# OpenBMB/VisRAG

Hardware: NVIDIA H100
Metric: page-images encoded/sec (higher is better)
Workload: dtype bf16

## Files before the change

visrag_b200/csrc/attention.cu:

```cuda
#include <string.h>
#include "common.h"
#include "attention.cuh"

namespace vr {

static int g_variant = 0;

template <int HS, bool CAUSAL, int NWG, bool F16>
static int launch_attention(const vr_attn_params& p, cudaStream_t stream) {
    using Cfg = AttCfg<HS, NWG>;
    AttMaps maps;
    memset(&maps, 0, sizeof(maps));
    const uint64_t qcols = p.ldq, kcols = p.ldk, vcols = p.ldv;
    if (int rc = make_tmap_2d(&maps.q64, p.q, p.q_rows, qcols, p.ldq, Cfg::BM, 64, 128, !F16)) return rc;
    if (int rc = make_tmap_2d(&maps.k64, p.k, p.kv_rows, kcols, p.ldk, ATT_BN, 64, 128, !F16)) return rc;
    if (int rc = make_tmap_2d(&maps.v64, p.v, p.kv_rows, vcols, p.ldv, ATT_BN, 64, 128, !F16)) return rc;
    if (Cfg::HAS16) {
        if (int rc = make_tmap_2d(&maps.q16, p.q, p.q_rows, qcols, p.ldq, Cfg::BM, 16, 32, !F16)) return rc;
        if (int rc = make_tmap_2d(&maps.k16, p.k, p.kv_rows, kcols, p.ldk, ATT_BN, 16, 32, !F16)) return rc;
        if (int rc = make_tmap_2d(&maps.v16, p.v, p.kv_rows, vcols, p.ldv, ATT_BN, 16, 32, !F16)) return rc;
    }
    AttArgs a;
    a.q_col0 = p.q_col0; a.k_col0 = p.k_col0; a.v_col0 = p.v_col0;
    a.head_dim = p.head_dim; a.heads = p.heads; a.batch = p.batch;
    a.cu_q = p.cu_q; a.cu_k = p.cu_k; a.max_q = p.max_q;
    a.scale_log2 = p.scale * 1.4426950408889634f;
    a.out = p.out;
    a.ldo = p.ldo;
    auto kern = attention_wgmma_kernel<HS, CAUSAL, NWG, F16>;
    static unsigned long long attr_set = 0;
    if (first_use_on_device(&attr_set))
        VR_CHECK_CUDA(cudaFuncSetAttribute(kern, cudaFuncAttributeMaxDynamicSharedMemorySize, Cfg::SMEM_BYTES));
    dim3 grid((p.max_q + Cfg::BM - 1) / Cfg::BM, p.heads, p.batch);
    kern<<<grid, Cfg::THREADS, Cfg::SMEM_BYTES, stream>>>(maps, a);
    VR_CHECK_CUDA(cudaGetLastError());
    return 0;
}

template <int HS, bool F16>
static int dispatch_attention(const vr_attn_params& p, cudaStream_t s) {
    const bool two = p.max_q > 64 && g_variant != 1;
    if (p.causal) return two ? launch_attention<HS, true, 2, F16>(p, s) : launch_attention<HS, true, 1, F16>(p, s);
    return two ? launch_attention<HS, false, 2, F16>(p, s) : launch_attention<HS, false, 1, F16>(p, s);
}

template <int HS>
static int dispatch_attention(const vr_attn_params& p, cudaStream_t s) {
    return (p.flags & VR_ATTN_F16) ? dispatch_attention<HS, true>(p, s) : dispatch_attention<HS, false>(p, s);
}

}

extern "C" void vr_attention_force_v1(int32_t variant) { vr::g_variant = variant; }

extern "C" int vr_attention(const vr_attn_params* p, void* stream) {
    using namespace vr;
    VR_REQUIRE(p && p->q && p->k && p->v && p->out && p->cu_k, "vr_attention: null pointer argument");
    VR_REQUIRE(p->heads > 0 && p->batch > 0 && p->max_q > 0 && p->max_k > 0, "vr_attention: empty problem");
    VR_REQUIRE(p->batch <= 65535 && p->heads <= 65535, "vr_attention: batch/heads exceed grid limits");
    VR_REQUIRE(p->head_dim <= p->head_stride && p->head_dim % 8 == 0, "vr_attention: head_dim %d vs stride %d",
               p->head_dim, p->head_stride);
    VR_REQUIRE(p->ldo % 8 == 0, "vr_attention: ldo must be a multiple of 8");
    VR_REQUIRE(!(p->flags & VR_ATTN_V_ONES_COLUMN) || p->head_dim == p->head_stride - 8,
               "vr_attention: VR_ATTN_V_ONES_COLUMN needs head_dim == head_stride - 8 (got %d / %d)", p->head_dim, p->head_stride);
    VR_REQUIRE_ALIGNED("vr_attention", "q", p->q, 16);
    VR_REQUIRE_ALIGNED("vr_attention", "k", p->k, 16);
    VR_REQUIRE_ALIGNED("vr_attention", "v", p->v, 16);
    VR_REQUIRE_ALIGNED("vr_attention", "cu_q", p->cu_q, 4);
    VR_REQUIRE_ALIGNED("vr_attention", "cu_k", p->cu_k, 4);
    VR_REQUIRE_ALIGNED("vr_attention", "out", p->out, 4);
    cudaStream_t s = reinterpret_cast<cudaStream_t>(stream);
    switch (p->head_stride) {
        case 64: return dispatch_attention<64>(*p, s);
        case 80: return dispatch_attention<80>(*p, s);
        case 128: return dispatch_attention<128>(*p, s);
        default: set_error("vr_attention: head_stride must be 64, 80 or 128 (got %d)", p->head_stride); return 2;
    }
}
```

visrag_b200/csrc/attention.cuh:

```cuda
#pragma once
#include "ptx.cuh"
#include "../../include/visrag_b200.h"

namespace vr {

constexpr int ATT_BN = 128;
constexpr int ATT_STAGES = 2;

template <int HS, int NWG>
struct AttCfg {
    static constexpr int BM = 64 * NWG;
    static constexpr int THREADS = 384;
    static constexpr int NCH = HS / 64;
    static constexpr bool HAS16 = (HS % 64) == 16;
    static_assert(HS == 64 || HS == 80 || HS == 128, "head stride must be 64, 80 or 128");
    static constexpr int Q_CHUNK = BM * 128;
    static constexpr int Q_BYTES = NCH * Q_CHUNK + (HAS16 ? BM * 32 : 0);
    static constexpr int TILE_BYTES = NCH * 16384 + (HAS16 ? 4096 : 0);
    static constexpr int OFF_Q = 0;
    static constexpr int OFF_K = (Q_BYTES + 1023) & ~1023;
    static constexpr int OFF_V = OFF_K + ATT_STAGES * TILE_BYTES;
    static constexpr int OFF_BAR = OFF_V + ATT_STAGES * TILE_BYTES;
    static constexpr int SMEM_BYTES = OFF_BAR + 128 + 1024;
};

struct AttArgs {
    int q_col0, k_col0, v_col0;
    int head_dim;
    int heads, batch;
    const int* cu_q;
    const int* cu_k;
    int max_q;
    float scale_log2;
    void* out;
    long long ldo;
};

struct AttMaps {
    CUtensorMap q64, q16, k64, k16, v64, v16;
};

template <bool F16, int NCH, bool HAS16>
__device__ __forceinline__ void att_store(const AttArgs& a, const float (&o)[NCH][32], const float (&o16)[8], float l_a, float l_b,
                                          int row_a, int len_q, int q_begin, int b, int head, int q4) {
    l_a += __shfl_xor_sync(0xffffffffu, l_a, 1);
    l_a += __shfl_xor_sync(0xffffffffu, l_a, 2);
    l_b += __shfl_xor_sync(0xffffffffu, l_b, 1);
    l_b += __shfl_xor_sync(0xffffffffu, l_b, 2);
#pragma unroll
    for (int half = 0; half < 2; ++half) {
        const int q_idx = row_a + 8 * half;
        if (q_idx >= len_q) continue;
        const float inv = 1.0f / (half ? l_b : l_a);
        const long long row = a.cu_q ? (long long)(q_begin + q_idx) : (long long)b * a.max_q + q_idx;
        half16_t<F16>* dst = reinterpret_cast<half16_t<F16>*>(a.out) + row * a.ldo + head * a.head_dim;
#pragma unroll
        for (int c = 0; c < NCH; ++c)
#pragma unroll
            for (int j = 0; j < 8; ++j) {
                const int col = c * 64 + j * 8 + q4 * 2;
                if (col < a.head_dim)
                    *reinterpret_cast<uint32_t*>(dst + col) = pack16x2<F16>(o[c][4 * j + 2 * half] * inv, o[c][4 * j + 2 * half + 1] * inv);
            }
        if (HAS16) {
#pragma unroll
            for (int j = 0; j < 2; ++j) {
                const int col = NCH * 64 + j * 8 + q4 * 2;
                if (col < a.head_dim)
                    *reinterpret_cast<uint32_t*>(dst + col) = pack16x2<F16>(o16[4 * j + 2 * half] * inv, o16[4 * j + 2 * half + 1] * inv);
            }
        }
    }
}

__device__ __forceinline__ void att_softmax_tile(float (&s)[64], float c, float& m_a, float& m_b, float& l_a, float& l_b,
                                                 float& alpha_a, float& alpha_b) {
    float mt_a = m_a, mt_b = m_b;
#pragma unroll
    for (int j = 0; j < 16; ++j) {
        mt_a = fmaxf(mt_a, fmaxf(s[4 * j], s[4 * j + 1]));
        mt_b = fmaxf(mt_b, fmaxf(s[4 * j + 2], s[4 * j + 3]));
    }
    mt_a = fmaxf(mt_a, __shfl_xor_sync(0xffffffffu, mt_a, 1));
    mt_a = fmaxf(mt_a, __shfl_xor_sync(0xffffffffu, mt_a, 2));
    mt_b = fmaxf(mt_b, __shfl_xor_sync(0xffffffffu, mt_b, 1));
    mt_b = fmaxf(mt_b, __shfl_xor_sync(0xffffffffu, mt_b, 2));
    const float mc_a = mt_a == -INFINITY ? 0.f : __fmul_rn(mt_a, c), mc_b = mt_b == -INFINITY ? 0.f : __fmul_rn(mt_b, c);
    alpha_a = ex2_ftz(__fmul_rn(m_a, c) - mc_a);
    alpha_b = ex2_ftz(__fmul_rn(m_b, c) - mc_b);
    m_a = mt_a;
    m_b = mt_b;
    float lt_a = 0.f, lt_b = 0.f;
#pragma unroll
    for (int j = 0; j < 16; ++j) {
#pragma unroll
        for (int e = 0; e < 2; ++e) {
            s[4 * j + e] = ex2_ftz(__fmaf_rn(s[4 * j + e], c, -mc_a));
            s[4 * j + 2 + e] = ex2_ftz(__fmaf_rn(s[4 * j + 2 + e], c, -mc_b));
            lt_a += s[4 * j + e];
            lt_b += s[4 * j + 2 + e];
        }
    }
    l_a = l_a * alpha_a + lt_a;
    l_b = l_b * alpha_b + lt_b;
}

template <int HS, bool CAUSAL, int NWG, bool F16>
__global__ void __launch_bounds__(384, 1)
attention_wgmma_kernel(const __grid_constant__ AttMaps maps, const AttArgs a) {
    using Cfg = AttCfg<HS, NWG>;
    constexpr int NCH = Cfg::NCH;
    extern __shared__ uint8_t smem_raw[];
    uint8_t* smem = reinterpret_cast<uint8_t*>((reinterpret_cast<uintptr_t>(smem_raw) + 1023) & ~uintptr_t(1023));
    uint8_t* sQ = smem + Cfg::OFF_Q;
    uint8_t* sK = smem + Cfg::OFF_K;
    uint8_t* sV = smem + Cfg::OFF_V;
    uint64_t* bars = reinterpret_cast<uint64_t*>(smem + Cfg::OFF_BAR);
    uint64_t* q_bar = bars + 0;
    uint64_t* k_full = bars + 1;
    uint64_t* k_empty = k_full + ATT_STAGES;
    uint64_t* v_full = k_empty + ATT_STAGES;
    uint64_t* v_empty = v_full + ATT_STAGES;
    uint64_t* v_tail = v_empty + ATT_STAGES;

    const int wg = threadIdx.x >> 7;
    const int warp = (threadIdx.x >> 5) & 3;
    const int lane = threadIdx.x & 31;
    const int qt = blockIdx.x, head = blockIdx.y, b = blockIdx.z;

    const int k_begin = a.cu_k[b];
    const int len_k = a.cu_k[b + 1] - k_begin;
    const int q_begin = a.cu_q ? a.cu_q[b] : 0;
    const int len_q = a.cu_q ? a.cu_q[b + 1] - q_begin : a.max_q;
    const int q0 = qt * Cfg::BM;
    if (q0 >= len_q || len_k <= 0) return;

    int nkt = (len_k + ATT_BN - 1) / ATT_BN;
    if (CAUSAL) {
        const int last_q = min(q0 + Cfg::BM, len_q) - 1;
        const int max_key = last_q + (len_k - len_q);
        nkt = min(nkt, max_key / ATT_BN + 1);
    }

    if (threadIdx.x == 0) {
        mbar_init(q_bar, 1);
        for (int i = 0; i < ATT_STAGES; ++i) {
            mbar_init(&k_full[i], 1);
            mbar_init(&v_full[i], 1);
            mbar_init(&k_empty[i], NWG * 4);
            mbar_init(&v_empty[i], NWG * 4);
        }
        mbar_init(v_tail, 1);
        fence_mbar_init();
    }
    __syncthreads();

    if (wg == 0 || wg > NWG) {
        setmaxnreg_dec<40>();
        if (wg == 0 && warp == 0) {
            const int tail = len_k - (nkt - 1) * ATT_BN;
            const int st_last = (nkt - 1) % ATT_STAGES;
            if (lane == 0) {
                const int qcol = a.q_col0 + head * HS, kcol = a.k_col0 + head * HS, vcol = a.v_col0 + head * HS;
                mbar_expect_tx(q_bar, Cfg::Q_BYTES);
#pragma unroll
                for (int c = 0; c < NCH; ++c) tma_load_2d(&maps.q64, q_bar, sQ + c * Cfg::Q_CHUNK, qcol + c * 64, q_begin + q0);
                if (Cfg::HAS16) tma_load_2d(&maps.q16, q_bar, sQ + NCH * Cfg::Q_CHUNK, qcol + NCH * 64, q_begin + q0);
                auto load_tile = [&](const CUtensorMap* m64, const CUtensorMap* m16, uint64_t* bar, uint8_t* dst, int col, int row) {
                    mbar_expect_tx(bar, Cfg::TILE_BYTES);
#pragma unroll
                    for (int c = 0; c < NCH; ++c) tma_load_2d(m64, bar, dst + c * 16384, col + c * 64, row);
                    if (Cfg::HAS16) tma_load_2d(m16, bar, dst + NCH * 16384, col + NCH * 64, row);
                };
                for (int kt = 0; kt < nkt; ++kt) {
                    const int st = kt % ATT_STAGES;
                    const uint32_t ph = (kt / ATT_STAGES) & 1;
                    mbar_wait(&k_empty[st], ph ^ 1);
                    load_tile(&maps.k64, &maps.k16, &k_full[st], sK + st * Cfg::TILE_BYTES, kcol, k_begin + kt * ATT_BN);
                    mbar_wait(&v_empty[st], ph ^ 1);
                    load_tile(&maps.v64, &maps.v16, kt == nkt - 1 && tail < ATT_BN ? v_tail : &v_full[st],
                              sV + st * Cfg::TILE_BYTES, vcol, k_begin + kt * ATT_BN);
                }
            }
            __syncwarp();
            if (tail < ATT_BN) {
                uint8_t* dst = sV + st_last * Cfg::TILE_BYTES;
                const uint4 zero = make_uint4(0u, 0u, 0u, 0u);
                mbar_wait(v_tail, 0);
#pragma unroll
                for (int c = 0; c < NCH; ++c)
                    for (int i = tail * 8 + lane; i < ATT_BN * 8; i += 32) reinterpret_cast<uint4*>(dst + c * 16384)[i] = zero;
                if (Cfg::HAS16)
                    for (int i = tail * 2 + lane; i < ATT_BN * 2; i += 32) reinterpret_cast<uint4*>(dst + NCH * 16384)[i] = zero;
                fence_proxy_async_smem();
                __syncwarp();
                if (lane == 0) mbar_arrive(&v_full[st_last]);
            }
        }
        return;
    }

    setmaxnreg_inc<232>();
    const int cw = wg - 1;
    const int g8 = lane >> 2, q4 = lane & 3;
    const int row_a = q0 + cw * 64 + warp * 16 + g8;
    const int row_b = row_a + 8;
    const int causal_shift = len_k - len_q;
    const uint32_t q_addr = smem_u32(sQ) + cw * (64 * 128);
    const uint32_t q16_addr = smem_u32(sQ) + NCH * Cfg::Q_CHUNK + cw * (64 * 32);

    if constexpr (NWG == 2 && HS != 128) {
        const float c = a.scale_log2;
        float o[NCH][32];
        float o16[8];
#pragma unroll
        for (int cc = 0; cc < NCH; ++cc)
#pragma unroll
            for (int j = 0; j < 32; ++j) o[cc][j] = 0.f;
#pragma unroll
        for (int j = 0; j < 8; ++j) o16[j] = 0.f;
        float m_a = -INFINITY, m_b = -INFINITY, l_a = 0.f, l_b = 0.f, alpha_a, alpha_b;
        float s[64];
        uint32_t pa[ATT_BN / 16][4];

        auto issue_s = [&](int kt) {
            const uint32_t k_addr = smem_u32(sK) + (kt % ATT_STAGES) * Cfg::TILE_BYTES;
#pragma unroll
            for (int cc = 0; cc < NCH; ++cc) {
#pragma unroll
                for (int kk = 0; kk < 4; ++kk)
                    wgmma_ss<F16, false>(s, make_smem_desc(q_addr + cc * Cfg::Q_CHUNK + kk * 32, 16, 1024, kLayoutSW128),
                                           make_smem_desc(k_addr + cc * 16384 + kk * 32, 16, 1024, kLayoutSW128), (cc | kk) != 0,
                                           std::integral_constant<int, 128>());
            }
            if (Cfg::HAS16)
                wgmma_ss<F16, false>(s, make_smem_desc(q16_addr, 16, 256, kLayoutSW32),
                                       make_smem_desc(k_addr + NCH * 16384, 16, 256, kLayoutSW32), 1, std::integral_constant<int, 128>());
            wgmma_commit();
        };
        auto issue_pv = [&](int kt) {
            const uint32_t v_addr = smem_u32(sV) + (kt % ATT_STAGES) * Cfg::TILE_BYTES;
#pragma unroll
            for (int kk = 0; kk < ATT_BN / 16; ++kk) {
#pragma unroll
                for (int cc = 0; cc < NCH; ++cc)
                    wgmma_rs_tb<F16>(o[cc], pa[kk], make_smem_desc(v_addr + cc * 16384 + kk * 2048, 16, 1024, kLayoutSW128), 1,
                                std::integral_constant<int, 64>());
                if (Cfg::HAS16)
                    wgmma_rs_tb<F16>(o16, pa[kk], make_smem_desc(v_addr + NCH * 16384 + kk * 512, 16, 256, kLayoutSW32), 1,
                                std::integral_constant<int, 16>());
            }
            wgmma_commit();
        };
        const int row0 = q0 + cw * 64;
        auto softmax = [&](int kt) {
            const int key0 = kt * ATT_BN;
            const bool full = key0 + ATT_BN <= len_k && (!CAUSAL || key0 + ATT_BN - 1 <= row0 + causal_shift);
            if (!full) {
                int lim_a = len_k - key0, lim_b = lim_a;
                if (CAUSAL) {
                    lim_a = min(lim_a, row_a + causal_shift - key0 + 1);
                    lim_b = min(lim_b, row_b + causal_shift - key0 + 1);
                }
#pragma unroll
                for (int j = 0; j < 16; ++j) {
#pragma unroll
                    for (int e = 0; e < 2; ++e) {
                        const int key = j * 8 + q4 * 2 + e;
                        s[4 * j + e] = key < lim_a ? s[4 * j + e] : -INFINITY;
                        s[4 * j + 2 + e] = key < lim_b ? s[4 * j + 2 + e] : -INFINITY;
                    }
                }
            }
            att_softmax_tile(s, c, m_a, m_b, l_a, l_b, alpha_a, alpha_b);
        };
        auto pack_p = [&] {
#pragma unroll
            for (int kk = 0; kk < ATT_BN / 16; ++kk) {
                pa[kk][0] = pack16x2<F16>(s[8 * kk + 0], s[8 * kk + 1]);
                pa[kk][1] = pack16x2<F16>(s[8 * kk + 2], s[8 * kk + 3]);
                pa[kk][2] = pack16x2<F16>(s[8 * kk + 4], s[8 * kk + 5]);
                pa[kk][3] = pack16x2<F16>(s[8 * kk + 6], s[8 * kk + 7]);
            }
        };
        auto rescale_o = [&] {
#pragma unroll
            for (int cc = 0; cc < NCH; ++cc)
#pragma unroll
                for (int j = 0; j < 8; ++j) {
                    o[cc][4 * j] *= alpha_a; o[cc][4 * j + 1] *= alpha_a;
                    o[cc][4 * j + 2] *= alpha_b; o[cc][4 * j + 3] *= alpha_b;
                }
            if (Cfg::HAS16) {
#pragma unroll
                for (int j = 0; j < 2; ++j) {
                    o16[4 * j] *= alpha_a; o16[4 * j + 1] *= alpha_a;
                    o16[4 * j + 2] *= alpha_b; o16[4 * j + 3] *= alpha_b;
                }
            }
        };
        auto turn_wait = [&] { named_bar_sync(1 + cw, 256); };
        auto turn_pass = [&] { named_bar_arrive(2 - cw, 256); };
        if (cw == 1) named_bar_arrive(1, 256);

        mbar_wait(q_bar, 0);
        mbar_wait(&k_full[0], 0);
        turn_wait();
        wgmma_fence();
        issue_s(0);
        turn_pass();
        wgmma_wait<0>();
        if (lane == 0) mbar_arrive(&k_empty[0]);
        wgmma_touch(s);
        softmax(0);
        pack_p();
        for (int kt = 0; kt + 1 < nkt; ++kt) {
            const int st = kt % ATT_STAGES, st1 = (kt + 1) % ATT_STAGES;
            mbar_wait(&k_full[st1], ((kt + 1) / ATT_STAGES) & 1);
            mbar_wait(&v_full[st], (kt / ATT_STAGES) & 1);
            turn_wait();
            wgmma_fence();
            issue_s(kt + 1);
            issue_pv(kt);
            turn_pass();
            wgmma_wait<1>();
            if (lane == 0) mbar_arrive(&k_empty[st1]);
            wgmma_touch(s);
            softmax(kt + 1);
            wgmma_wait<0>();
            if (lane == 0) mbar_arrive(&v_empty[st]);
#pragma unroll
            for (int cc = 0; cc < NCH; ++cc) wgmma_touch(o[cc]);
            wgmma_touch(o16);
            rescale_o();
            pack_p();
        }
        {
            const int kt = nkt - 1, st = kt % ATT_STAGES;
            mbar_wait(&v_full[st], (kt / ATT_STAGES) & 1);
            turn_wait();
            wgmma_fence();
            issue_pv(kt);
            turn_pass();
            wgmma_wait<0>();
            if (lane == 0) mbar_arrive(&v_empty[st]);
#pragma unroll
            for (int cc = 0; cc < NCH; ++cc) wgmma_touch(o[cc]);
            wgmma_touch(o16);
        }
        if (cw == 0) turn_wait();
        att_store<F16, NCH, Cfg::HAS16>(a, o, o16, l_a, l_b, row_a, len_q, q_begin, b, head, q4);
    } else {
        float o[NCH][32];
        float o16[8];
#pragma unroll
        for (int c = 0; c < NCH; ++c)
#pragma unroll
            for (int j = 0; j < 32; ++j) o[c][j] = 0.f;
#pragma unroll
        for (int j = 0; j < 8; ++j) o16[j] = 0.f;
        float m_a = -INFINITY, m_b = -INFINITY, l_a = 0.f, l_b = 0.f;

        mbar_wait(q_bar, 0);
        for (int kt = 0; kt < nkt; ++kt) {
            const int st = kt % ATT_STAGES;
            const uint32_t ph = (kt / ATT_STAGES) & 1;
            const uint32_t k_addr = smem_u32(sK) + st * Cfg::TILE_BYTES, v_addr = smem_u32(sV) + st * Cfg::TILE_BYTES;
            float s[64];
            mbar_wait(&k_full[st], ph);
            wgmma_fence();
#pragma unroll
            for (int c = 0; c < NCH; ++c) {
#pragma unroll
                for (int kk = 0; kk < 4; ++kk)
                    wgmma_ss<F16, false>(s, make_smem_desc(q_addr + c * Cfg::Q_CHUNK + kk * 32, 16, 1024, kLayoutSW128),
                                           make_smem_desc(k_addr + c * 16384 + kk * 32, 16, 1024, kLayoutSW128), (c | kk) != 0,
                                           std::integral_constant<int, 128>());
            }
            if (Cfg::HAS16)
                wgmma_ss<F16, false>(s, make_smem_desc(q16_addr, 16, 256, kLayoutSW32),
                                       make_smem_desc(k_addr + NCH * 16384, 16, 256, kLayoutSW32), 1, std::integral_constant<int, 128>());
            wgmma_commit();
            wgmma_wait<0>();
            if (lane == 0) mbar_arrive(&k_empty[st]);
            wgmma_touch(s);

            const int key0 = kt * ATT_BN;
            int lim_a = len_k - key0, lim_b = lim_a;
            if (CAUSAL) {
                lim_a = min(lim_a, row_a + causal_shift - key0 + 1);
                lim_b = min(lim_b, row_b + causal_shift - key0 + 1);
            }
#pragma unroll
            for (int j = 0; j < 16; ++j) {
#pragma unroll
                for (int e = 0; e < 2; ++e) {
                    const int key = j * 8 + q4 * 2 + e;
                    s[4 * j + e] = key < lim_a ? s[4 * j + e] : -INFINITY;
                    s[4 * j + 2 + e] = key < lim_b ? s[4 * j + 2 + e] : -INFINITY;
                }
            }
            float alpha_a, alpha_b;
            att_softmax_tile(s, a.scale_log2, m_a, m_b, l_a, l_b, alpha_a, alpha_b);
#pragma unroll
            for (int c = 0; c < NCH; ++c)
#pragma unroll
                for (int j = 0; j < 8; ++j) {
                    o[c][4 * j] *= alpha_a; o[c][4 * j + 1] *= alpha_a;
                    o[c][4 * j + 2] *= alpha_b; o[c][4 * j + 3] *= alpha_b;
                }
            if (Cfg::HAS16) {
#pragma unroll
                for (int j = 0; j < 2; ++j) {
                    o16[4 * j] *= alpha_a; o16[4 * j + 1] *= alpha_a;
                    o16[4 * j + 2] *= alpha_b; o16[4 * j + 3] *= alpha_b;
                }
            }
            uint32_t pa[ATT_BN / 16][4];
#pragma unroll
            for (int kk = 0; kk < ATT_BN / 16; ++kk) {
                pa[kk][0] = pack16x2<F16>(s[8 * kk + 0], s[8 * kk + 1]);
                pa[kk][1] = pack16x2<F16>(s[8 * kk + 2], s[8 * kk + 3]);
                pa[kk][2] = pack16x2<F16>(s[8 * kk + 4], s[8 * kk + 5]);
                pa[kk][3] = pack16x2<F16>(s[8 * kk + 6], s[8 * kk + 7]);
            }
            mbar_wait(&v_full[st], ph);
            wgmma_fence();
#pragma unroll
            for (int kk = 0; kk < ATT_BN / 16; ++kk) {
#pragma unroll
                for (int c = 0; c < NCH; ++c) {
                    wgmma_rs_tb<F16>(o[c], pa[kk], make_smem_desc(v_addr + c * 16384 + kk * 2048, 16, 1024, kLayoutSW128), 1,
                                std::integral_constant<int, 64>());
                }
                if (Cfg::HAS16) {
                    wgmma_rs_tb<F16>(o16, pa[kk], make_smem_desc(v_addr + NCH * 16384 + kk * 512, 16, 256, kLayoutSW32), 1,
                                std::integral_constant<int, 16>());
                }
            }
            wgmma_commit();
            wgmma_wait<0>();
            if (lane == 0) mbar_arrive(&v_empty[st]);
#pragma unroll
            for (int c = 0; c < NCH; ++c) wgmma_touch(o[c]);
            wgmma_touch(o16);
        }

        att_store<F16, NCH, Cfg::HAS16>(a, o, o16, l_a, l_b, row_a, len_q, q_begin, b, head, q4);
    }
}

}
```

Baseline: 337.3.

## Add persistent attention kernel overlapping epilogue with next tile's QK

Replaces the two-warpgroup ping-pong path for head strides 64/80 with a persistent kernel launched with one CTA per SM. Each CTA loops over (q-tile, head, batch) work items, double-buffers Q and uses a 3-stage K/V ring. It issues the next item's first QK^T during the current item's last PV, so the store epilogue and prologue overlap with tensor-core work. This removes per-block launch and tail cost, but adds more complex barrier and phase bookkeeping and changes the smem footprint.

```diff
diff --git a/visrag_b200/csrc/attention.cu b/visrag_b200/csrc/attention.cu
--- a/visrag_b200/csrc/attention.cu
+++ b/visrag_b200/csrc/attention.cu
@@ -27,12 +27,23 @@
     a.scale_log2 = p.scale * 1.4426950408889634f;
     a.out = p.out;
     a.ldo = p.ldo;
-    auto kern = attention_wgmma_kernel<HS, CAUSAL, NWG, F16>;
-    static unsigned long long attr_set = 0;
-    if (first_use_on_device(&attr_set))
-        VR_CHECK_CUDA(cudaFuncSetAttribute(kern, cudaFuncAttributeMaxDynamicSharedMemorySize, Cfg::SMEM_BYTES));
-    dim3 grid((p.max_q + Cfg::BM - 1) / Cfg::BM, p.heads, p.batch);
-    kern<<<grid, Cfg::THREADS, Cfg::SMEM_BYTES, stream>>>(maps, a);
+    const int q_tiles = (p.max_q + Cfg::BM - 1) / Cfg::BM;
+    if constexpr (NWG == 2 && HS != 128) {
+        using PCfg = AttCfg<HS, 2, 2, ATT_PSTAGES>;
+        auto kern = attention_persistent_kernel<HS, CAUSAL, F16>;
+        static unsigned long long attr_set = 0;
+        if (first_use_on_device(&attr_set))
+            VR_CHECK_CUDA(cudaFuncSetAttribute(kern, cudaFuncAttributeMaxDynamicSharedMemorySize, PCfg::SMEM_BYTES));
+        const long long items = static_cast<long long>(q_tiles) * p.heads * p.batch;
+        const int grid = items < num_sms() ? static_cast<int>(items) : num_sms();
+        kern<<<grid, PCfg::THREADS, PCfg::SMEM_BYTES, stream>>>(maps, a);
+    } else {
+        auto kern = attention_wgmma_kernel<HS, CAUSAL, NWG, F16>;
+        static unsigned long long attr_set = 0;
+        if (first_use_on_device(&attr_set))
+            VR_CHECK_CUDA(cudaFuncSetAttribute(kern, cudaFuncAttributeMaxDynamicSharedMemorySize, Cfg::SMEM_BYTES));
+        kern<<<dim3(q_tiles, p.heads, p.batch), Cfg::THREADS, Cfg::SMEM_BYTES, stream>>>(maps, a);
+    }
     VR_CHECK_CUDA(cudaGetLastError());
     return 0;
 }
diff --git a/visrag_b200/csrc/attention.cuh b/visrag_b200/csrc/attention.cuh
--- a/visrag_b200/csrc/attention.cuh
+++ b/visrag_b200/csrc/attention.cuh
@@ -6,8 +6,9 @@
 
 constexpr int ATT_BN = 128;
 constexpr int ATT_STAGES = 2;
-
-template <int HS, int NWG>
+constexpr int ATT_PSTAGES = 3;
+
+template <int HS, int NWG, int QBUF = 1, int STAGES = ATT_STAGES>
 struct AttCfg {
     static constexpr int BM = 64 * NWG;
     static constexpr int THREADS = 384;
@@ -16,12 +17,16 @@
     static_assert(HS == 64 || HS == 80 || HS == 128, "head stride must be 64, 80 or 128");
     static constexpr int Q_CHUNK = BM * 128;
     static constexpr int Q_BYTES = NCH * Q_CHUNK + (HAS16 ? BM * 32 : 0);
+    static constexpr int Q_STRIDE = (Q_BYTES + 1023) & ~1023;
     static constexpr int TILE_BYTES = NCH * 16384 + (HAS16 ? 4096 : 0);
     static constexpr int OFF_Q = 0;
-    static constexpr int OFF_K = (Q_BYTES + 1023) & ~1023;
-    static constexpr int OFF_V = OFF_K + ATT_STAGES * TILE_BYTES;
-    static constexpr int OFF_BAR = OFF_V + ATT_STAGES * TILE_BYTES;
-    static constexpr int SMEM_BYTES = OFF_BAR + 128 + 1024;
+    static constexpr int OFF_K = QBUF * Q_STRIDE;
+    static constexpr int OFF_V = OFF_K + STAGES * TILE_BYTES;
+    static constexpr int OFF_BAR = OFF_V + STAGES * TILE_BYTES;
+    static constexpr int BAR_BYTES = 2 * QBUF + 5 * STAGES <= 16 ? 128 : 256;
+    static constexpr int SMEM_BYTES = OFF_BAR + BAR_BYTES + 1024;
+    static_assert(8 * (2 * QBUF + 5 * STAGES) <= BAR_BYTES, "mbarriers do not fit");
+    static_assert(SMEM_BYTES <= 227 * 1024, "over the 227 KB shared-memory limit");
 };
 
 struct AttArgs {
@@ -209,148 +214,7 @@
     const uint32_t q_addr = smem_u32(sQ) + cw * (64 * 128);
     const uint32_t q16_addr = smem_u32(sQ) + NCH * Cfg::Q_CHUNK + cw * (64 * 32);
 
-    if constexpr (NWG == 2 && HS != 128) {
-        const float c = a.scale_log2;
-        float o[NCH][32];
-        float o16[8];
-#pragma unroll
-        for (int cc = 0; cc < NCH; ++cc)
-#pragma unroll
-            for (int j = 0; j < 32; ++j) o[cc][j] = 0.f;
-#pragma unroll
-        for (int j = 0; j < 8; ++j) o16[j] = 0.f;
-        float m_a = -INFINITY, m_b = -INFINITY, l_a = 0.f, l_b = 0.f, alpha_a, alpha_b;
-        float s[64];
-        uint32_t pa[ATT_BN / 16][4];
-
-        auto issue_s = [&](int kt) {
-            const uint32_t k_addr = smem_u32(sK) + (kt % ATT_STAGES) * Cfg::TILE_BYTES;
-#pragma unroll
-            for (int cc = 0; cc < NCH; ++cc) {
-#pragma unroll
-                for (int kk = 0; kk < 4; ++kk)
-                    wgmma_ss<F16, false>(s, make_smem_desc(q_addr + cc * Cfg::Q_CHUNK + kk * 32, 16, 1024, kLayoutSW128),
-                                           make_smem_desc(k_addr + cc * 16384 + kk * 32, 16, 1024, kLayoutSW128), (cc | kk) != 0,
-                                           std::integral_constant<int, 128>());
-            }
-            if (Cfg::HAS16)
-                wgmma_ss<F16, false>(s, make_smem_desc(q16_addr, 16, 256, kLayoutSW32),
-                                       make_smem_desc(k_addr + NCH * 16384, 16, 256, kLayoutSW32), 1, std::integral_constant<int, 128>());
-            wgmma_commit();
-        };
-        auto issue_pv = [&](int kt) {
-            const uint32_t v_addr = smem_u32(sV) + (kt % ATT_STAGES) * Cfg::TILE_BYTES;
-#pragma unroll
-            for (int kk = 0; kk < ATT_BN / 16; ++kk) {
-#pragma unroll
-                for (int cc = 0; cc < NCH; ++cc)
-                    wgmma_rs_tb<F16>(o[cc], pa[kk], make_smem_desc(v_addr + cc * 16384 + kk * 2048, 16, 1024, kLayoutSW128), 1,
-                                std::integral_constant<int, 64>());
-                if (Cfg::HAS16)
-                    wgmma_rs_tb<F16>(o16, pa[kk], make_smem_desc(v_addr + NCH * 16384 + kk * 512, 16, 256, kLayoutSW32), 1,
-                                std::integral_constant<int, 16>());
-            }
-            wgmma_commit();
-        };
-        const int row0 = q0 + cw * 64;
-        auto softmax = [&](int kt) {
-            const int key0 = kt * ATT_BN;
-            const bool full = key0 + ATT_BN <= len_k && (!CAUSAL || key0 + ATT_BN - 1 <= row0 + causal_shift);
-            if (!full) {
-                int lim_a = len_k - key0, lim_b = lim_a;
-                if (CAUSAL) {
-                    lim_a = min(lim_a, row_a + causal_shift - key0 + 1);
-                    lim_b = min(lim_b, row_b + causal_shift - key0 + 1);
-                }
-#pragma unroll
-                for (int j = 0; j < 16; ++j) {
-#pragma unroll
-                    for (int e = 0; e < 2; ++e) {
-                        const int key = j * 8 + q4 * 2 + e;
-                        s[4 * j + e] = key < lim_a ? s[4 * j + e] : -INFINITY;
-                        s[4 * j + 2 + e] = key < lim_b ? s[4 * j + 2 + e] : -INFINITY;
-                    }
-                }
-            }
-            att_softmax_tile(s, c, m_a, m_b, l_a, l_b, alpha_a, alpha_b);
-        };
-        auto pack_p = [&] {
-#pragma unroll
-            for (int kk = 0; kk < ATT_BN / 16; ++kk) {
-                pa[kk][0] = pack16x2<F16>(s[8 * kk + 0], s[8 * kk + 1]);
-                pa[kk][1] = pack16x2<F16>(s[8 * kk + 2], s[8 * kk + 3]);
-                pa[kk][2] = pack16x2<F16>(s[8 * kk + 4], s[8 * kk + 5]);
-                pa[kk][3] = pack16x2<F16>(s[8 * kk + 6], s[8 * kk + 7]);
-            }
-        };
-        auto rescale_o = [&] {
-#pragma unroll
-            for (int cc = 0; cc < NCH; ++cc)
-#pragma unroll
-                for (int j = 0; j < 8; ++j) {
-                    o[cc][4 * j] *= alpha_a; o[cc][4 * j + 1] *= alpha_a;
-                    o[cc][4 * j + 2] *= alpha_b; o[cc][4 * j + 3] *= alpha_b;
-                }
-            if (Cfg::HAS16) {
-#pragma unroll
-                for (int j = 0; j < 2; ++j) {
-                    o16[4 * j] *= alpha_a; o16[4 * j + 1] *= alpha_a;
-                    o16[4 * j + 2] *= alpha_b; o16[4 * j + 3] *= alpha_b;
-                }
-            }
-        };
-        auto turn_wait = [&] { named_bar_sync(1 + cw, 256); };
-        auto turn_pass = [&] { named_bar_arrive(2 - cw, 256); };
-        if (cw == 1) named_bar_arrive(1, 256);
-
-        mbar_wait(q_bar, 0);
-        mbar_wait(&k_full[0], 0);
-        turn_wait();
-        wgmma_fence();
-        issue_s(0);
-        turn_pass();
-        wgmma_wait<0>();
-        if (lane == 0) mbar_arrive(&k_empty[0]);
-        wgmma_touch(s);
-        softmax(0);
-        pack_p();
-        for (int kt = 0; kt + 1 < nkt; ++kt) {
-            const int st = kt % ATT_STAGES, st1 = (kt + 1) % ATT_STAGES;
-            mbar_wait(&k_full[st1], ((kt + 1) / ATT_STAGES) & 1);
-            mbar_wait(&v_full[st], (kt / ATT_STAGES) & 1);
-            turn_wait();
-            wgmma_fence();
-            issue_s(kt + 1);
-            issue_pv(kt);
-            turn_pass();
-            wgmma_wait<1>();
-            if (lane == 0) mbar_arrive(&k_empty[st1]);
-            wgmma_touch(s);
-            softmax(kt + 1);
-            wgmma_wait<0>();
-            if (lane == 0) mbar_arrive(&v_empty[st]);
-#pragma unroll
-            for (int cc = 0; cc < NCH; ++cc) wgmma_touch(o[cc]);
-            wgmma_touch(o16);
-            rescale_o();
-            pack_p();
-        }
-        {
-            const int kt = nkt - 1, st = kt % ATT_STAGES;
-            mbar_wait(&v_full[st], (kt / ATT_STAGES) & 1);
-            turn_wait();
-            wgmma_fence();
-            issue_pv(kt);
-            turn_pass();
-            wgmma_wait<0>();
-            if (lane == 0) mbar_arrive(&v_empty[st]);
-#pragma unroll
-            for (int cc = 0; cc < NCH; ++cc) wgmma_touch(o[cc]);
-            wgmma_touch(o16);
-        }
-        if (cw == 0) turn_wait();
-        att_store<F16, NCH, Cfg::HAS16>(a, o, o16, l_a, l_b, row_a, len_q, q_begin, b, head, q4);
-    } else {
+    {
         float o[NCH][32];
         float o16[8];
 #pragma unroll
@@ -450,4 +314,321 @@
     }
 }
 
+struct AttItem {
+    int q0, head, b;
+    int q_begin, len_q, k_begin, len_k;
+    int nkt;
+};
+
+template <bool CAUSAL>
+__device__ __forceinline__ bool att_item(const AttArgs& a, int q_tiles, long long w, AttItem& it) {
+    const long long hq = w / q_tiles;
+    it.q0 = static_cast<int>(w - hq * q_tiles) * 128;
+    it.head = static_cast<int>(hq % a.heads);
+    it.b = static_cast<int>(hq / a.heads);
+    it.k_begin = a.cu_k[it.b];
+    it.len_k = a.cu_k[it.b + 1] - it.k_begin;
+    it.q_begin = a.cu_q ? a.cu_q[it.b] : 0;
+    it.len_q = a.cu_q ? a.cu_q[it.b + 1] - it.q_begin : a.max_q;
+    if (it.q0 >= it.len_q || it.len_k <= 0) return false;
+    it.nkt = (it.len_k + ATT_BN - 1) / ATT_BN;
+    if (CAUSAL) {
+        const int last_q = min(it.q0 + 128, it.len_q) - 1;
+        const int max_key = last_q + (it.len_k - it.len_q);
+        it.nkt = max(1, min(it.nkt, max_key / ATT_BN + 1));
+    }
+    return true;
 }
+
+template <int HS, bool CAUSAL, bool F16>
+__global__ void __launch_bounds__(384, 1)
+attention_persistent_kernel(const __grid_constant__ AttMaps maps, const AttArgs a) {
+    using Cfg = AttCfg<HS, 2, 2, ATT_PSTAGES>;
+    constexpr int NCH = Cfg::NCH;
+    constexpr int STAGES = ATT_PSTAGES;
+    extern __shared__ uint8_t smem_raw[];
+    uint8_t* smem = reinterpret_cast<uint8_t*>((reinterpret_cast<uintptr_t>(smem_raw) + 1023) & ~uintptr_t(1023));
+    uint8_t* sQ = smem + Cfg::OFF_Q;
+    uint8_t* sK = smem + Cfg::OFF_K;
+    uint8_t* sV = smem + Cfg::OFF_V;
+    uint64_t* bars = reinterpret_cast<uint64_t*>(smem + Cfg::OFF_BAR);
+    uint64_t* q_full = bars + 0;
+    uint64_t* q_empty = q_full + 2;
+    uint64_t* k_full = q_empty + 2;
+    uint64_t* k_empty = k_full + STAGES;
+    uint64_t* v_full = k_empty + STAGES;
+    uint64_t* v_empty = v_full + STAGES;
+    uint64_t* v_tail = v_empty + STAGES;
+
+    const int wg = threadIdx.x >> 7;
+    const int warp = (threadIdx.x >> 5) & 3;
+    const int lane = threadIdx.x & 31;
+    const int q_tiles = (a.max_q + Cfg::BM - 1) / Cfg::BM;
+    const long long items = static_cast<long long>(q_tiles) * a.heads * a.batch;
+
+    if (threadIdx.x == 0) {
+        for (int i = 0; i < 2; ++i) {
+            mbar_init(&q_full[i], 1);
+            mbar_init(&q_empty[i], 8);
+        }
+        for (int i = 0; i < STAGES; ++i) {
+            mbar_init(&k_full[i], 1);
+            mbar_init(&v_full[i], 1);
+            mbar_init(&k_empty[i], 8);
+            mbar_init(&v_empty[i], 8);
+            mbar_init(&v_tail[i], 1);
+        }
+        fence_mbar_init();
+    }
+    __syncthreads();
+
+    if (wg == 0) {
+        setmaxnreg_dec<40>();
+        if (warp == 0 && lane == 0) {
+            auto load_tile = [&](const CUtensorMap* m64, const CUtensorMap* m16, uint64_t* bar, uint8_t* dst, int col, int row) {
+                mbar_expect_tx(bar, Cfg::TILE_BYTES);
+#pragma unroll
+                for (int c = 0; c < NCH; ++c) tma_load_2d(m64, bar, dst + c * 16384, col + c * 64, row);
+                if (Cfg::HAS16) tma_load_2d(m16, bar, dst + NCH * 16384, col + NCH * 64, row);
+            };
+            uint32_t qi = 0, kv = 0;
+            for (long long w = blockIdx.x; w < items; w += gridDim.x) {
+                AttItem it;
+                if (!att_item<CAUSAL>(a, q_tiles, w, it)) continue;
+                const int qcol = a.q_col0 + it.head * HS, kcol = a.k_col0 + it.head * HS, vcol = a.v_col0 + it.head * HS;
+                const int qs = qi & 1;
+                uint8_t* dq = sQ + qs * Cfg::Q_STRIDE;
+                mbar_wait(&q_empty[qs], ((qi >> 1) & 1) ^ 1);
+                mbar_expect_tx(&q_full[qs], Cfg::Q_BYTES);
+#pragma unroll
+                for (int c = 0; c < NCH; ++c) tma_load_2d(&maps.q64, &q_full[qs], dq + c * Cfg::Q_CHUNK, qcol + c * 64, it.q_begin + it.q0);
+                if (Cfg::HAS16) tma_load_2d(&maps.q16, &q_full[qs], dq + NCH * Cfg::Q_CHUNK, qcol + NCH * 64, it.q_begin + it.q0);
+                const int tail = it.len_k - (it.nkt - 1) * ATT_BN;
+                for (int kt = 0; kt < it.nkt; ++kt, ++kv) {
+                    const int st = kv % STAGES;
+                    const uint32_t ph = (kv / STAGES) & 1;
+                    mbar_wait(&k_empty[st], ph ^ 1);
+                    load_tile(&maps.k64, &maps.k16, &k_full[st], sK + st * Cfg::TILE_BYTES, kcol, it.k_begin + kt * ATT_BN);
+                    mbar_wait(&v_empty[st], ph ^ 1);
+                    load_tile(&maps.v64, &maps.v16, kt == it.nkt - 1 && tail < ATT_BN ? &v_tail[st] : &v_full[st],
+                              sV + st * Cfg::TILE_BYTES, vcol, it.k_begin + kt * ATT_BN);
+                }
+                ++qi;
+            }
+        } else if (warp == 1) {
+            uint32_t kv = 0, tail_ph = 0;
+            for (long long w = blockIdx.x; w < items; w += gridDim.x) {
+                AttItem it;
+                if (!att_item<CAUSAL>(a, q_tiles, w, it)) continue;
+                kv += it.nkt;
+                const int tail = it.len_k - (it.nkt - 1) * ATT_BN;
+                if (tail >= ATT_BN) continue;
+                const int st = (kv - 1) % STAGES;
+                uint8_t* dst = sV + st * Cfg::TILE_BYTES;
+                const uint4 zero = make_uint4(0u, 0u, 0u, 0u);
+                mbar_wait(&v_tail[st], (tail_ph >> st) & 1);
+                tail_ph ^= 1u << st;
+#pragma unroll
+                for (int c = 0; c < NCH; ++c)
+                    for (int i = tail * 8 + lane; i < ATT_BN * 8; i += 32) reinterpret_cast<uint4*>(dst + c * 16384)[i] = zero;
+                if (Cfg::HAS16)
+                    for (int i = tail * 2 + lane; i < ATT_BN * 2; i += 32) reinterpret_cast<uint4*>(dst + NCH * 16384)[i] = zero;
+                fence_proxy_async_smem();
+                __syncwarp();
+                if (lane == 0) mbar_arrive(&v_full[st]);
+            }
+        }
+        return;
+    }
+
+    setmaxnreg_inc<232>();
+    const int cw = wg - 1;
+    const int g8 = lane >> 2, q4 = lane & 3;
+    const int row_in = cw * 64 + warp * 16 + g8;
+    const float c = a.scale_log2;
+    float o[NCH][32];
+    float o16[8];
+    auto zero_o = [&] {
+#pragma unroll
+        for (int cc = 0; cc < NCH; ++cc)
+#pragma unroll
+            for (int j = 0; j < 32; ++j) o[cc][j] = 0.f;
+#pragma unroll
+        for (int j = 0; j < 8; ++j) o16[j] = 0.f;
+    };
+    zero_o();
+    float m_a = -INFINITY, m_b = -INFINITY, l_a = 0.f, l_b = 0.f, alpha_a, alpha_b;
+    float s[64];
+    uint32_t pa[ATT_BN / 16][4];
+
+    auto issue_s = [&](uint32_t qs, uint32_t kv) {
+        const uint32_t q_addr = smem_u32(sQ) + qs * Cfg::Q_STRIDE + cw * (64 * 128);
+        const uint32_t q16_addr = smem_u32(sQ) + qs * Cfg::Q_STRIDE + NCH * Cfg::Q_CHUNK + cw * (64 * 32);
+        const uint32_t k_addr = smem_u32(sK) + (kv % STAGES) * Cfg::TILE_BYTES;
+#pragma unroll
+        for (int cc = 0; cc < NCH; ++cc) {
+#pragma unroll
+            for (int kk = 0; kk < 4; ++kk)
+                wgmma_ss<F16, false>(s, make_smem_desc(q_addr + cc * Cfg::Q_CHUNK + kk * 32, 16, 1024, kLayoutSW128),
+                                       make_smem_desc(k_addr + cc * 16384 + kk * 32, 16, 1024, kLayoutSW128), (cc | kk) != 0,
+                                       std::integral_constant<int, 128>());
+        }
+        if (Cfg::HAS16)
+            wgmma_ss<F16, false>(s, make_smem_desc(q16_addr, 16, 256, kLayoutSW32),
+                                   make_smem_desc(k_addr + NCH * 16384, 16, 256, kLayoutSW32), 1, std::integral_constant<int, 128>());
+        wgmma_commit();
+    };
+    auto issue_pv = [&](uint32_t kv) {
+        const uint32_t v_addr = smem_u32(sV) + (kv % STAGES) * Cfg::TILE_BYTES;
+#pragma unroll
+        for (int kk = 0; kk < ATT_BN / 16; ++kk) {
+#pragma unroll
+            for (int cc = 0; cc < NCH; ++cc)
+                wgmma_rs_tb<F16>(o[cc], pa[kk], make_smem_desc(v_addr + cc * 16384 + kk * 2048, 16, 1024, kLayoutSW128), 1,
+                            std::integral_constant<int, 64>());
+            if (Cfg::HAS16)
+                wgmma_rs_tb<F16>(o16, pa[kk], make_smem_desc(v_addr + NCH * 16384 + kk * 512, 16, 256, kLayoutSW32), 1,
+                            std::integral_constant<int, 16>());
+        }
+        wgmma_commit();
+    };
+    auto softmax = [&](const AttItem& it, int kt) {
+        const int key0 = kt * ATT_BN;
+        const int causal_shift = it.len_k - it.len_q;
+        const int row0 = it.q0 + cw * 64;
+        const bool full = key0 + ATT_BN <= it.len_k && (!CAUSAL || key0 + ATT_BN - 1 <= row0 + causal_shift);
+        if (!full) {
+            const int row_a = it.q0 + row_in, row_b = row_a + 8;
+            int lim_a = it.len_k - key0, lim_b = lim_a;
+            if (CAUSAL) {
+                lim_a = min(lim_a, row_a + causal_shift - key0 + 1);
+                lim_b = min(lim_b, row_b + causal_shift - key0 + 1);
+            }
+#pragma unroll
+            for (int j = 0; j < 16; ++j) {
+#pragma unroll
+                for (int e = 0; e < 2; ++e) {
+                    const int key = j * 8 + q4 * 2 + e;
+                    s[4 * j + e] = key < lim_a ? s[4 * j + e] : -INFINITY;
+                    s[4 * j + 2 + e] = key < lim_b ? s[4 * j + 2 + e] : -INFINITY;
+                }
+            }
+        }
+        att_softmax_tile(s, c, m_a, m_b, l_a, l_b, alpha_a, alpha_b);
+    };
+    auto pack_p = [&] {
+#pragma unroll
+        for (int kk = 0; kk < ATT_BN / 16; ++kk) {
+            pa[kk][0] = pack16x2<F16>(s[8 * kk + 0], s[8 * kk + 1]);
+            pa[kk][1] = pack16x2<F16>(s[8 * kk + 2], s[8 * kk + 3]);
+            pa[kk][2] = pack16x2<F16>(s[8 * kk + 4], s[8 * kk + 5]);
+            pa[kk][3] = pack16x2<F16>(s[8 * kk + 6], s[8 * kk + 7]);
+        }
+    };
+    auto rescale_o = [&] {
+#pragma unroll
+        for (int cc = 0; cc < NCH; ++cc)
+#pragma unroll
+            for (int j = 0; j < 8; ++j) {
+                o[cc][4 * j] *= alpha_a; o[cc][4 * j + 1] *= alpha_a;
+                o[cc][4 * j + 2] *= alpha_b; o[cc][4 * j + 3] *= alpha_b;
+            }
+        if (Cfg::HAS16) {
+#pragma unroll
+            for (int j = 0; j < 2; ++j) {
+                o16[4 * j] *= alpha_a; o16[4 * j + 1] *= alpha_a;
+                o16[4 * j + 2] *= alpha_b; o16[4 * j + 3] *= alpha_b;
+            }
+        }
+    };
+    auto touch_o = [&] {
+#pragma unroll
+        for (int cc = 0; cc < NCH; ++cc) wgmma_touch(o[cc]);
+        wgmma_touch(o16);
+    };
+
+    long long w = blockIdx.x;
+    AttItem cur;
+    while (w < items && !att_item<CAUSAL>(a, q_tiles, w, cur)) w += gridDim.x;
+    if (w >= items) return;
+
+    auto turn_wait = [&] { named_bar_sync(1 + cw, 256); };
+    auto turn_pass = [&] { named_bar_arrive(2 - cw, 256); };
+    if (cw == 1) named_bar_arrive(1, 256);
+
+    uint32_t qi = 0, kv = 0;
+    mbar_wait(&q_full[0], 0);
+    mbar_wait(&k_full[0], 0);
+    turn_wait();
+    wgmma_fence();
+    issue_s(0, 0);
+    turn_pass();
+    wgmma_wait<0>();
+    if (lane == 0) mbar_arrive(&k_empty[0]);
+    wgmma_touch(s);
+    softmax(cur, 0);
+    pack_p();
+    for (;;) {
+        long long wn = w + gridDim.x;
+        AttItem nxt;
+        while (wn < items && !att_item<CAUSAL>(a, q_tiles, wn, nxt)) wn += gridDim.x;
+        const bool more = wn < items;
+        const int nk = more ? cur.nkt : cur.nkt - 1;
+        for (int kt = 0; kt < nk; ++kt, ++kv) {
+            const bool last = kt + 1 == cur.nkt;
+            const uint32_t st = kv % STAGES, st1 = (kv + 1) % STAGES;
+            const uint32_t qs = (last ? qi + 1 : qi) & 1;
+            if (last) mbar_wait(&q_full[qs], ((qi + 1) >> 1) & 1);
+            mbar_wait(&k_full[st1], ((kv + 1) / STAGES) & 1);
+            mbar_wait(&v_full[st], (kv / STAGES) & 1);
+            turn_wait();
+            wgmma_fence();
+            issue_s(qs, kv + 1);
+            issue_pv(kv);
+            turn_pass();
+            const float lp_a = l_a, lp_b = l_b;
+            wgmma_wait<1>();
+            if (lane == 0) {
+                mbar_arrive(&k_empty[st1]);
+                if (last) mbar_arrive(&q_empty[qi & 1]);
+            }
+            wgmma_touch(s);
+            if (last) {
+                m_a = m_b = -INFINITY;
+                l_a = l_b = 0.f;
+                softmax(nxt, 0);
+            } else {
+                softmax(cur, kt + 1);
+            }
+            wgmma_wait<0>();
+            if (lane == 0) mbar_arrive(&v_empty[st]);
+            touch_o();
+            if (last) {
+                att_store<F16, NCH, Cfg::HAS16>(a, o, o16, lp_a, lp_b, cur.q0 + row_in, cur.len_q, cur.q_begin, cur.b, cur.head, q4);
+                zero_o();
+            } else {
+                rescale_o();
+            }
+            pack_p();
+        }
+        if (!more) break;
+        cur = nxt;
+        w = wn;
+        ++qi;
+    }
+    {
+        const uint32_t st = kv % STAGES;
+        mbar_wait(&v_full[st], (kv / STAGES) & 1);
+        turn_wait();
+        wgmma_fence();
+        issue_pv(kv);
+        turn_pass();
+        wgmma_wait<0>();
+        if (lane == 0) mbar_arrive(&v_empty[st]);
+        touch_o();
+    }
+    if (cw == 0) turn_wait();
+    att_store<F16, NCH, Cfg::HAS16>(a, o, o16, l_a, l_b, cur.q0 + row_in, cur.len_q, cur.q_begin, cur.b, cur.head, q4);
+}
+
+}
```

Result: no change. 338.5 (median of 6 runs) (+0.3%).
